# JCBrouwer/maua-style

Hardware: AMD Instinct MI355X
Metric: optimizer iterations/sec at 1024x1024 VGG-19 (higher is better)
Workload: dtype f32 (fp16x3 split-precision MFMA, fp32 accumulate)

## Files before the change

maua-style_amd/csrc/conv_x3p.hip:

```cpp
#include <stdlib.h>

#include <type_traits>

#include "conv_host.hpp"
#include "fp16x3.hpp"

namespace maua {

constexpr int XP_COT = 64;
constexpr int XP_ROWS = 16, XP_PR = 18, XP_PC = 34;
constexpr int XP_NPOS = XP_PR * XP_PC;
constexpr int XP_NPOS_PAD = 624;
constexpr int XP_PLANE = XP_NPOS_PAD * 16;
constexpr int XP_PATCH_BYTES = 8 * XP_PLANE;
constexpr int XP_TAP_BYTES = 2 * 4 * XP_COT * 16;
constexpr int XP_W_BYTES = 9 * XP_TAP_BYTES;
constexpr int XP_NI = 5;
constexpr int XP_THREADS = 512;
constexpr int XP_BIAS_MAX = 512;
constexpr int XP_LDS_BYTES = XP_PATCH_BYTES + XP_W_BYTES + 64 + XP_BIAS_MAX * 4 + XP_THREADS * 12;
constexpr unsigned XP_OOB = 0x80000000u;
#ifndef XP_W1_PIECES
#define XP_W1_PIECES 4
#endif
#ifndef XP_EARLY_LOADS
#define XP_EARLY_LOADS 0
#endif
#ifndef XP_MIDFOLD
#define XP_MIDFOLD 1
#endif
#ifndef XP_STAGGER
#define XP_STAGGER 0
#endif

__host__ __device__ constexpr int xp_first_pieces(bool pool) { return pool ? XP_W1_PIECES / 2 : XP_W1_PIECES; }
__host__ __device__ constexpr int xp_step_of(bool pool, int k) {
    const int p1 = xp_first_pieces(pool);
    return pool ? (k < p1 ? 16 - 2 * (p1 - 1 - k) : 20 + 2 * (k - p1)) : (k < p1 ? 17 - p1 + k : 20 + (k - p1));
}

struct X3pArgs {
    int items;
    int tiles;
    int ncot;
    int ksplit;
    int cps;
    int nmain;
    int n2;
    int groups;
    int tiles_y;
    int d_split, d_tx, d_ty, d_cot, d_n;
    int order;
    float w_inv_scale;
};

#ifdef XP_STAMP
#define XP_MARK(k)                                                                                                       \
    do {                                                                                                                 \
        if (lane == 0 && p.mask && chunk_no < 60) {                                                                      \
            const_cast<float*>(p.mask)[(((int64_t)blockIdx.x * 8 + wave) * 64 + chunk_no) * 8 + (k)] =                   \
                __builtin_bit_cast(float, (unsigned)__builtin_amdgcn_s_memtime());                                       \
        }                                                                                                                \
    } while (0)
#else
#define XP_MARK(k) do {} while (0)
#endif

#define XP_FENCE() __builtin_amdgcn_sched_barrier(0)

#define XP_PIPE_PLAIN(VA)                                             \
    do {                                                              \
        _Pragma("unroll") for (int m_ = 0; m_ < 12; ++m_) {           \
            __builtin_amdgcn_sched_group_barrier(0x008, 1, 0);        \
            __builtin_amdgcn_sched_group_barrier(0x100, 1, 0);        \
            __builtin_amdgcn_sched_group_barrier(0x020, 1, 0);        \
            __builtin_amdgcn_sched_group_barrier(0x200, 1, 0);        \
            __builtin_amdgcn_sched_group_barrier(0x002, VA, 0);       \
        }                                                             \
    } while (0)
#define XP_PIPE(VA)                                                   \
    do {                                                              \
        _Pragma("unroll") for (int m_ = 0; m_ < 12; ++m_) {           \
            __builtin_amdgcn_sched_group_barrier(0x008, 1, 0);        \
            __builtin_amdgcn_sched_group_barrier(0x100, 1, 0);        \
            __builtin_amdgcn_sched_group_barrier(0x020, 1, 0);        \
            __builtin_amdgcn_sched_group_barrier(0x040, 1, 0);        \
            __builtin_amdgcn_sched_group_barrier(0x200, 1, 0);        \
            __builtin_amdgcn_sched_group_barrier(0x002, VA, 0);       \
        }                                                             \
    } while (0)

template <bool OM, bool POOL, bool UNPOOL, bool GRAM>
__global__ void __launch_bounds__(XP_THREADS, 2) conv_x3p_kernel(ConvArgs p, X3pArgs q) {
    extern __shared__ __attribute__((aligned(16))) unsigned char smem[];
    unsigned char* Pl = smem;
    unsigned char* Wl = smem + XP_PATCH_BYTES;
    float* Ml = reinterpret_cast<float*>(smem + XP_PATCH_BYTES + XP_W_BYTES);
    float* Bl = Ml + 16;
    unsigned* Tl = reinterpret_cast<unsigned*>(Bl + XP_BIAS_MAX);

    const int tid = threadIdx.x;
    const int lane = tid & 63, wave = tid >> 6;
    const int px = lane & 15, oct = lane >> 4;
    const int wv = __builtin_amdgcn_readfirstlane(wave);
    auto my_tid = [&]() {
        int t = tid;
        asm volatile("" : "+v"(t));
        return t;
    };
    const float w_inv_scale = q.w_inv_scale;
    const int ksplit = q.ksplit;
    const bool slab = ksplit > 1;
    const int in_plane = p.H * p.W;
    const int out_plane = p.OH * p.OW;
    const int st_w = UNPOOL ? p.W >> 1 : p.W;
    const int st_plane = UNPOOL ? (p.H >> 1) * (p.W >> 1) : in_plane;
    const unsigned code_mask = (unsigned)p.in_code_mask;

    const int stride = q.groups >> 3;
    const int band_begin = (int)((int64_t)(blockIdx.x & 7) * q.items / 8), band_end = (int)((int64_t)((blockIdx.x & 7) + 1) * q.items / 8);
    const int gq = (int)(blockIdx.x & 7) * stride + (int)(blockIdx.x >> 3);
    const int item_begin = band_begin + (int)(blockIdx.x >> 3), item_end = band_end;
    if (item_begin >= item_end) return;
    if (XP_STAGGER > 0)
        for (int i = 0; i < (gq & 3) * XP_STAGGER; ++i) __builtin_amdgcn_s_sleep(16);
    struct Item {
        int n, cot, split, x0, y0, cb, ce;
    };
    const int tiles_w = p.tiles_x * 32, tiles_h = (q.tiles / p.tiles_x) * XP_ROWS;
    auto chunk_range = [&](Item& it) {
        it.cb = it.split * q.cps;
        it.ce = min(q.nmain, it.cb + q.cps);
    };
    auto decode = [&](int idx) {
        Item it;
        int t = idx;
        it.split = t % ksplit;
        t /= ksplit;
        int tile;
        if (q.order) {
            it.cot = t % q.ncot;
            t /= q.ncot;
            tile = t % q.tiles;
            it.n = t / q.tiles;
        } else {
            tile = t % q.tiles;
            t /= q.tiles;
            it.cot = t % q.ncot;
            it.n = t / q.ncot;
        }
        it.x0 = (tile % p.tiles_x) * 32;
        it.y0 = (tile / p.tiles_x) * XP_ROWS;
        it.n = __builtin_amdgcn_readfirstlane(it.n);
        it.cot = __builtin_amdgcn_readfirstlane(it.cot);
        it.split = __builtin_amdgcn_readfirstlane(it.split);
        it.x0 = __builtin_amdgcn_readfirstlane(it.x0);
        it.y0 = __builtin_amdgcn_readfirstlane(it.y0);
        chunk_range(it);
        return it;
    };
    auto advance = [&](Item it) {
        int c;
        it.split += q.d_split;
        c = it.split >= ksplit ? 1 : 0;
        it.split -= c ? ksplit : 0;
        if (q.order) {
            it.cot += q.d_cot + c;
            c = it.cot >= q.ncot ? 1 : 0;
            it.cot -= c ? q.ncot : 0;
        }
        it.x0 += (q.d_tx + c) * 32;
        c = it.x0 >= tiles_w ? 1 : 0;
        it.x0 -= c ? tiles_w : 0;
        it.y0 += (q.d_ty + c) * XP_ROWS;
        c = it.y0 >= tiles_h ? 1 : 0;
        it.y0 -= c ? tiles_h : 0;
        if (!q.order) {
            it.cot += q.d_cot + c;
            c = it.cot >= q.ncot ? 1 : 0;
            it.cot -= c ? q.ncot : 0;
        }
        it.n += q.d_n + c;
        chunk_range(it);
        return it;
    };

    constexpr int NI = UNPOOL ? 2 : XP_NI;
    constexpr int NV = 2;
    unsigned voff[NV];
    unsigned lds_w[2] = {0u, 0u};
    unsigned vcode[UNPOOL ? 2 : 1], inmask[UNPOOL ? 2 : 1];
    if constexpr (UNPOOL) {
        constexpr int PR = XP_ROWS / 2 + 2, PCW = 18;
#pragma unroll
        for (int k = 0; k < 2; ++k) {
            const int idx = tid + XP_THREADS * k;
            const int o = idx / (PR * PCW);
            const int rem = idx - o * PR * PCW;
            const int pr = rem / PCW, pc = rem - pr * PCW;
            Tl[k * XP_THREADS + tid] = (unsigned)(pr | pc << 8 | o << 16 | (idx < 4 * PR * PCW ? 1 << 24 : 0));
        }
    } else {
        const int ra = tid / XP_PC, ca = tid - ra * XP_PC;
        Tl[tid] = (unsigned)(ra | ca << 8 | 1 << 24);
        const int o4 = tid / 100, pb = 512 + tid - o4 * 100;
        const int rb = pb / XP_PC, cb4 = pb - rb * XP_PC;
        Tl[XP_THREADS + tid] = (unsigned)(rb | cb4 << 8 | o4 << 16 | (tid < 400 ? 1 << 24 : 0));
        vcode[0] = inmask[0] = 0;
    }
    auto set_tile = [&](int x0, int y0) {
        const int tid = my_tid();
        if constexpr (UNPOOL) {
#pragma unroll
            for (int k = 0; k < NI; ++k) {
                const unsigned wh = Tl[k * XP_THREADS + tid];
                const int pr = (int)(wh & 0xffu), pc = (int)((wh >> 8) & 0xffu), o = (int)((wh >> 16) & 0xffu);
                const bool item = (wh >> 24) != 0;
                const int ppy = ((y0 - p.pad) >> 1) + pr, ppx = ((x0 - p.pad) >> 1) + pc;
                const bool ok = item & ((unsigned)ppy < (unsigned)(p.H >> 1)) & ((unsigned)ppx < (unsigned)st_w);
                const int pidx = ppy * st_w + ppx;
                voff[k] = ok ? (unsigned)(o * 8 * st_plane + pidx) * 4u : XP_OOB;
                vcode[k] = ok ? (unsigned)(o * st_plane + pidx) * 8u : XP_OOB;
                const int r0 = 2 * ppy - (y0 - p.pad), c0 = 2 * ppx - (x0 - p.pad);
                inmask[k] = 0;
#pragma unroll
                for (int qd = 0; qd < 4; ++qd) {
                    const int r = r0 + (qd >> 1), c = c0 + (qd & 1);
                    inmask[k] |= (item & ((unsigned)r < (unsigned)XP_PR) & ((unsigned)c < (unsigned)XP_PC)) ? 1u << qd : 0u;
                }
                lds_w[k] = (unsigned)(o * XP_PLANE + (r0 * XP_PC + c0) * 16);
            }
        } else {
#pragma unroll
            for (int k = 0; k < 2; ++k) {
                const unsigned wh = Tl[k * XP_THREADS + tid];
                const int r = (int)(wh & 0xffu), c = (int)((wh >> 8) & 0xffu), o = (int)((wh >> 16) & 0xffu);
                const int iy = y0 + r - p.pad, ix = x0 + c - p.pad;
                const bool ok = ((wh >> 24) != 0) & ((unsigned)iy < (unsigned)p.H) & ((unsigned)ix < (unsigned)p.W);
                const unsigned v = ok ? (unsigned)(o * 8 * in_plane + iy * p.W + ix) * 4u : XP_OOB;
                if (k == 0) voff[0] = v;
                else Tl[2 * XP_THREADS + tid] = v;
            }
        }
    };
    const unsigned range = (unsigned)st_plane * 128u;
    float rp[NI][8];
    u32x2 cd[NI];
    unsigned sel2[NI][4];
    struct PatchSrc {
        __amdgpu_buffer_rsrc_t x, codes;
    };
    auto patch_rsrc = [&](int n, int ch) {
        asm volatile("" : "+s"(ch));
        PatchSrc r;
        const int64_t first = ((int64_t)n * p.Cin + (int64_t)ch * 32) * st_plane;
        r.x = __builtin_amdgcn_make_buffer_rsrc(const_cast<float*>(p.x + first), 0, range, 0x00020000);
        r.codes = r.x;
        if constexpr (UNPOOL) r.codes = __builtin_amdgcn_make_buffer_rsrc(const_cast<unsigned char*>(p.in_codes + first), 0, range >> 2, 0x00020000);
        return r;
    };
    auto load_patch_part = [&](const PatchSrc& rs, int c_lo, int c_hi) {
        if constexpr (UNPOOL) {
            if (c_lo == 0) {
#pragma unroll
                for (int k = 0; k < NI; ++k) cd[k] = __builtin_amdgcn_raw_buffer_load_b64(rs.codes, vcode[k], 0, 0);
            }
#pragma unroll
            for (int c = c_lo; c < c_hi; ++c)
#pragma unroll
                for (int k = 0; k < NI; ++k)
                    rp[k][c] = __builtin_bit_cast(float, __builtin_amdgcn_raw_buffer_load_b32(rs.x, voff[k], c * st_plane * 4, 0));
        } else {
#pragma unroll
            for (int c = c_lo; c < c_hi; ++c)
#pragma unroll
                for (int k = 0; k < NI; ++k)
                    rp[k][c] = __builtin_bit_cast(float, __builtin_amdgcn_raw_buffer_load_b32(rs.x, k < 4 ? voff[0] : voff[1], ((k < 4 ? 8 * k : 0) + c) * st_plane * 4, 0));
        }
    };
    auto publish_max = [&]() {
        if constexpr (UNPOOL) {
            const unsigned m2 = code_mask * 0x00010001u;
#pragma unroll
            for (int k = 0; k < NI; ++k)
#pragma unroll
                for (int i = 0; i < 4; ++i) {
                    sel2[k][i] = __builtin_amdgcn_perm(0u, cd[k][i >> 1], (i & 1) ? 0x0c030c02u : 0x0c010c00u) & m2;
                    const unsigned s0 = sel2[k][i] & 0xffffu, s1 = sel2[k][i] >> 16;
                    rp[k][2 * i] = ((inmask[k] >> s0) & 1u) ? rp[k][2 * i] : 0.f;
                    rp[k][2 * i + 1] = ((inmask[k] >> s1) & 1u) ? rp[k][2 * i + 1] : 0.f;
                }
        }
        float m = 0.f;
#pragma unroll
        for (int k = 0; k < NI; ++k)
#pragma unroll
            for (int c = 0; c < 8; ++c) m = fmaxf(m, fabsf(rp[k][c]));
        m = wave_max_nonneg(m);
        if ((my_tid() & 63) == 0) Ml[wv] = m;
    };
    float sx = 1.f;
    auto chunk_scale = [&]() {
        const float m = fmaxf(fmaxf(fmaxf(Ml[0], Ml[1]), fmaxf(Ml[2], Ml[3])), fmaxf(fmaxf(Ml[4], Ml[5]), fmaxf(Ml[6], Ml[7])));
        int e = (int)((__builtin_bit_cast(unsigned, m) >> 23) & 0xffu) - 127;
        e = m > 0.f ? max(e, -100) : 11;
        e = __builtin_amdgcn_readfirstlane(e);
        sx = __builtin_bit_cast(float, (unsigned)(127 + 11 - e) << 23);
        return __builtin_bit_cast(float, (unsigned)(127 + e - 11) << 23);
    };
    auto split_item = [&](int k) {
        if (k >= NI) return;
#pragma unroll
        for (int c = 0; c < 8; ++c) asm volatile("" : "+v"(rp[k][c]));
        unsigned hu[4], lu[4];
#pragma unroll
        for (int qd = 0; qd < 4; ++qd) {
            const float v0 = rp[k][2 * qd], v1 = rp[k][2 * qd + 1];
            const f16x2 h2 = {(_Float16)(v0 * sx), (_Float16)(v1 * sx)};
            const f16x2 l2 = {(_Float16)fmaf(v0, sx, -(float)h2[0]), (_Float16)fmaf(v1, sx, -(float)h2[1])};
            hu[qd] = __builtin_bit_cast(unsigned, h2);
            lu[qd] = __builtin_bit_cast(unsigned, l2);
        }
#pragma unroll
        for (int qd = 0; qd < 4; ++qd) {
            rp[k][qd] = __builtin_bit_cast(float, hu[qd]);
            rp[k][4 + qd] = __builtin_bit_cast(float, lu[qd]);
        }
#pragma unroll
        for (int c = 0; c < 8; ++c) asm volatile("" : "+v"(rp[k][c]));
    };
    auto store_patch = [&]() {
        if constexpr (UNPOOL) {
#pragma unroll
            for (int k = 0; k < NI; ++k)
#pragma unroll
                for (int qd = 0; qd < 4; ++qd)
                    if ((inmask[k] >> qd) & 1u) {
                        const unsigned dst = lds_w[k] + (unsigned)(((qd >> 1) * XP_PC + (qd & 1)) * 16);
                        u32x4 h, l;
#pragma unroll
                        for (int i = 0; i < 4; ++i) {
                            const unsigned t = sel2[k][i] ^ ((unsigned)qd * 0x00010001u);
                            const unsigned keep = ((t & 0xffffu) ? 0u : 0xffffu) | ((t >> 16) ? 0u : 0xffff0000u);
                            h[i] = __builtin_bit_cast(unsigned, rp[k][i]) & keep;
                            l[i] = __builtin_bit_cast(unsigned, rp[k][4 + i]) & keep;
                        }
                        *reinterpret_cast<u32x4*>(Pl + dst) = h;
                        *reinterpret_cast<u32x4*>(Pl + 4 * XP_PLANE + dst) = l;
                    }
            return;
        }
        const int t_ = my_tid();
#pragma unroll
        for (int k = 0; k < NI; ++k) {
            const u32x4 h = {__builtin_bit_cast(unsigned, rp[k][0]), __builtin_bit_cast(unsigned, rp[k][1]), __builtin_bit_cast(unsigned, rp[k][2]),
                             __builtin_bit_cast(unsigned, rp[k][3])};
            const u32x4 l = {__builtin_bit_cast(unsigned, rp[k][4]), __builtin_bit_cast(unsigned, rp[k][5]), __builtin_bit_cast(unsigned, rp[k][6]),
                             __builtin_bit_cast(unsigned, rp[k][7])};
            unsigned dst = (unsigned)t_ * 16u + (unsigned)(XP_PLANE * k);
            if (k == NI - 1) {
                const unsigned wh = Tl[XP_THREADS + t_];
                dst = (wh >> 24) ? ((wh >> 16) & 0xffu) * XP_PLANE + ((wh & 0xffu) * XP_PC + ((wh >> 8) & 0xffu)) * 16u : (unsigned)(3 * XP_PLANE + (XP_NPOS_PAD - 1) * 16);
            }
            *reinterpret_cast<u32x4*>(Pl + dst) = h;
            *reinterpret_cast<u32x4*>(Pl + 4 * XP_PLANE + dst) = l;
        }
    };

    const unsigned char* __restrict__ bank = reinterpret_cast<const unsigned char*>(p.w6);
    const unsigned lane16 = lane * 16;
    auto dma_filters = [&](int ch, int cot, int first, int count, int i0 = 0) {
        const unsigned char* src = bank + ((int64_t)ch * q.ncot + cot) * XP_W_BYTES;
#pragma unroll
        for (int i = i0; i < i0 + count; ++i) {
            const int pl = first + wv + 8 * i;
            const unsigned char* g = src + pl * 1024;
            const unsigned lds_dst = (unsigned)(size_t)(__attribute__((address_space(3))) unsigned char*)(Wl + pl * 1024);
            unsigned keep;
            asm volatile("s_mov_b32 %0, m0\n\ts_mov_b32 m0, %2\n\ts_nop 0\n\tglobal_load_lds_dwordx4 %1, %3\n\ts_mov_b32 m0, %0"
                         : "=&s"(keep)
                         : "v"(lane16), "s"(__builtin_amdgcn_readfirstlane(lds_dst)), "s"(g)
                         : "memory");
        }
    };

    int b_base = oct * XP_PLANE + ((2 * wave) * XP_PC + px) * 16;
    int a_base = oct * 1024 + px * 16;

    f32x4 acc[4][4], master[4][4];
    f16x8 bf[4][2], af[2][2];
    auto load_bg = [&](int g, int part, int tap) {
        const int ky = tap / 3, kx = tap - 3 * ky;
        bf[g][part] = *reinterpret_cast<const f16x8*>(Pl + b_base + part * 4 * XP_PLANE + (((g >> 1) + ky) * XP_PC + (g & 1) * 16 + kx) * 16);
    };
    auto load_ai = [&](int buf, int tap, int i) {
#pragma unroll
        for (int part = 0; part < 2; ++part) af[buf][part] = *reinterpret_cast<const f16x8*>(Wl + a_base + (tap * 2 + part) * 4096 + i * 256);
    };
    auto step_ = [&](auto stores, int tap, int i, int next_tap, auto fresh, float inv, auto va, auto&& extra) {
        constexpr bool FRESH = decltype(fresh)::value;
        constexpr int VA = decltype(va)::value;
        const int cur = i & 1;
        const bool refresh = i == 3 && next_tap >= 0;
        XP_FENCE();
        if (i < 3) load_ai(cur ^ 1, tap, i + 1);
        else if (next_tap >= 0 && tap != 4) load_ai(cur ^ 1, next_tap, 0);
        const f32x4 zero = {0.f, 0.f, 0.f, 0.f};
        if constexpr (FRESH) {
#pragma unroll
            for (int g = 0; g < 4; ++g) asm volatile("" : "+v"(acc[i][g]));
#pragma unroll
            for (int g = 0; g < 4; ++g)
#pragma unroll
                for (int r = 0; r < 4; ++r) master[i][g][r] = fmaf(acc[i][g][r], inv, master[i][g][r]);
#pragma unroll
            for (int g = 0; g < 4; ++g) asm volatile("" : "+v"(master[i][g]));
        }
#pragma unroll
        for (int g = 0; g < 4; ++g) acc[i][g] = __builtin_amdgcn_mfma_f32_16x16x32_f16(af[cur][1], bf[g][0], FRESH ? zero : acc[i][g], 0, 0, 0);
#pragma unroll
        for (int g = 0; g < 4; ++g) {
            acc[i][g] = __builtin_amdgcn_mfma_f32_16x16x32_f16(af[cur][0], bf[g][0], acc[i][g], 0, 0, 0);
            if (refresh) load_bg(g, 0, next_tap);
        }
        extra();
#pragma unroll
        for (int g = 0; g < 4; ++g) {
            acc[i][g] = __builtin_amdgcn_mfma_f32_16x16x32_f16(af[cur][0], bf[g][1], acc[i][g], 0, 0, 0);
            if (refresh) load_bg(g, 1, next_tap);
        }
        if constexpr (decltype(stores)::value) XP_PIPE(VA);
        else XP_PIPE_PLAIN(VA);
        XP_FENCE();
    };
    auto nothing = []() {};
    constexpr std::true_type FOLD{};
    constexpr std::false_type KEEP{};
    constexpr std::integral_constant<int, 0> V0{};
    constexpr std::integral_constant<int, 2> V2{};
    constexpr std::integral_constant<int, 4> V4{};

    Item cur = decode(item_begin);
    Item fin = cur;
    bool fin_valid = false;
    __amdgpu_buffer_rsrc_t rs_out, rs_aux;
    unsigned so_base = 0;
    unsigned vo[2];
    bool row_ok[4] = {true, true, true, true};
    const int PW = p.OW >> 1;
    const int pplane = (p.OH >> 1) * PW;
    auto epi_begin = [&]() {
        const int t_ = my_tid();
        const int lane = t_ & 63, px = t_ & 15, oct = (t_ >> 4) & 3, wave = wv;
        if constexpr (POOL) {
            const int64_t img = (int64_t)fin.n * p.Cout * pplane;
            rs_out = __builtin_amdgcn_make_buffer_rsrc(p.y + img, 0, (unsigned)p.Cout * (unsigned)pplane * 4u, 0x00020000);
            rs_aux = __builtin_amdgcn_make_buffer_rsrc(p.pool_codes + img, 0, (unsigned)p.Cout * (unsigned)pplane, 0x00020000);
            so_base = (unsigned)((fin.y0 >> 1) * PW + (fin.x0 >> 1));
#pragma unroll
            for (int h = 0; h < 2; ++h) {
                const int oy = fin.y0 + 2 * wave, oxx = fin.x0 + 16 * h + px;
                const bool store = fin_valid && (lane & 1) == 0 && oy + 1 < p.OH && oxx + 1 < p.OW;
                vo[h] = store ? (unsigned)(wave * PW + ((16 * h + px) >> 1)) : XP_OOB;
            }
        } else {
            const int64_t img = (int64_t)fin.n * p.Cout * out_plane;
            float* base = slab ? p.ws + ((int64_t)fin.n * ksplit + fin.split) * p.Cout * out_plane : p.y + img;
            rs_out = __builtin_amdgcn_make_buffer_rsrc(base, 0, (unsigned)p.Cout * (unsigned)out_plane * 4u, 0x00020000);
            rs_aux = rs_out;
            if constexpr (OM) rs_aux = __builtin_amdgcn_make_buffer_rsrc(const_cast<float*>(p.omask + img), 0, (unsigned)p.Cout * (unsigned)out_plane * 4u, 0x00020000);
            so_base = (unsigned)((fin.cot * XP_COT) * out_plane + fin.y0 * p.OW + fin.x0) * 4u;
#pragma unroll
            for (int h = 0; h < 2; ++h)
                vo[h] = fin_valid && fin.x0 + 16 * h + px < p.OW ? (unsigned)((4 * oct) * out_plane + (2 * wave) * p.OW + 16 * h + px) * 4u : XP_OOB;
#pragma unroll
            for (int g = 0; g < 4; ++g) row_ok[g] = fin.y0 + 2 * wv + (g >> 1) < p.OH;
        }
    };
    float mk[2][4];
    auto epi_load = [&](int k) {
        if constexpr (OM) {
            const int i = k >> 2, g = k & 3;
            const unsigned v = row_ok[g] ? vo[g & 1] : XP_OOB;
#pragma unroll
            for (int r = 0; r < 4; ++r)
                mk[k % 2][r] = __builtin_bit_cast(float, __builtin_amdgcn_raw_buffer_load_b32(
                    rs_aux, v, so_base + (unsigned)((16 * i + r) * out_plane + (g >> 1) * p.OW) * 4u, 0));
        }
    };
    auto reset_group = [&](int i, int cot) {
        const int oct = (my_tid() >> 4) & 3;
        const f32x4 b = *reinterpret_cast<const f32x4*>(Bl + cot * XP_COT + 16 * i + 4 * oct);
#pragma unroll
        for (int g = 0; g < 4; ++g) master[i][g] = b;
    };
    auto epi_piece = [&](int k, int next_cot) {
        const int oct = (my_tid() >> 4) & 3;
        if constexpr (POOL) {
            if (k >= 8) return;
            const int i = k >> 1, h = k & 1;
            unsigned pk = 0;
            const unsigned so = (unsigned)((fin.cot * XP_COT + 16 * i) * pplane) + so_base;
#pragma unroll
            for (int r = 0; r < 4; ++r) {
                float a = master[i][h][r], c = master[i][2 + h][r];
                a = a > 0.f ? a : 0.f;
                c = c > 0.f ? c : 0.f;
                const float b = __builtin_bit_cast(float, __builtin_amdgcn_update_dpp(0, __builtin_bit_cast(int, a), 0x101, 0xf, 0xf, false));
                const float d = __builtin_bit_cast(float, __builtin_amdgcn_update_dpp(0, __builtin_bit_cast(int, c), 0x101, 0xf, 0xf, false));
                float m = a;
                unsigned arg = 0;
                if (b > m) { m = b; arg = 1; }
                if (c > m) { m = c; arg = 2; }
                if (d > m) { m = d; arg = 3; }
                pk |= (arg | (m > 0.f ? 0u : 4u)) << (8 * r);
                const unsigned v = vo[h] == XP_OOB ? XP_OOB : ((unsigned)(4 * oct * pplane) + vo[h]) * 4u;
                __builtin_amdgcn_raw_buffer_store_b32(__builtin_bit_cast(unsigned, m), rs_out, v, (so + (unsigned)(r * pplane)) * 4u, 0);
            }
            const unsigned vc = vo[h] == XP_OOB ? XP_OOB : ((unsigned)((oct >> 1) * pplane) + vo[h]) * 8u + 4u * (oct & 1);
            __builtin_amdgcn_raw_buffer_store_b32(pk, rs_aux, vc, ((unsigned)(((fin.cot * XP_COT + 16 * i) >> 3) * pplane) + so_base) * 8u, 0);
            if (h == 1) reset_group(i, next_cot);
        } else {
            const int i = k >> 2, g = k & 3;
            const unsigned v = row_ok[g] ? vo[g & 1] : XP_OOB;
#pragma unroll
            for (int r = 0; r < 4; ++r) {
                float val = master[i][g][r];
                if (p.relu && !slab) val = val > 0.f ? val : 0.f;
                if constexpr (OM) val = mk[k % 2][r] > 0.f ? val : 0.f;
                __builtin_amdgcn_raw_buffer_store_b32(__builtin_bit_cast(unsigned, val), rs_out, v,
                                                      so_base + (unsigned)((16 * i + r) * out_plane + (g >> 1) * p.OW) * 4u, 0);
            }
            if (g == 3) reset_group(i, next_cot);
        }
    };

    auto gram_phase = [&](const Item& it, float inv_pending) {
#pragma unroll
        for (int i = 0; i < 4; ++i)
#pragma unroll
            for (int g = 0; g < 4; ++g)
#pragma unroll
                for (int r = 0; r < 4; ++r) {
                    master[i][g][r] = fmaf(acc[i][g][r], inv_pending, master[i][g][r]);
                    acc[i][g][r] = 0.f;
                }
        const float d_inv_scale = p.dinv[it.n];
        const unsigned char* dbank = reinterpret_cast<const unsigned char*>(p.dbank);
        unsigned vf[4];
#pragma unroll
        for (int g = 0; g < 4; ++g) {
            const int oy = it.y0 + 2 * wave + (g >> 1), oxx = it.x0 + (g & 1) * 16 + px;
            vf[g] = (oy < p.OH && oxx < p.OW) ? (unsigned)((oct * 8) * out_plane + oy * p.OW + oxx) * 4u : XP_OOB;
        }
        const unsigned frange = (unsigned)out_plane * 128u;
        float f[4][8];
        auto request = [&](int c2) {
            asm volatile("" : "+s"(c2));
            const __amdgpu_buffer_rsrc_t rs = __builtin_amdgcn_make_buffer_rsrc(
                const_cast<float*>(p.omask + ((int64_t)it.n * p.Cout + (int64_t)c2 * 32) * out_plane), 0, frange, 0x00020000);
#pragma unroll
            for (int c = 0; c < 8; ++c)
#pragma unroll
                for (int g = 0; g < 4; ++g) f[g][c] = __builtin_bit_cast(float, __builtin_amdgcn_raw_buffer_load_b32(rs, vf[g], c * out_plane * 4, 0));
        };
        request(0);
        for (int c2 = 0; c2 < q.n2; ++c2) {
            float m = 0.f;
#pragma unroll
            for (int g = 0; g < 4; ++g)
#pragma unroll
                for (int c = 0; c < 8; ++c) m = fmaxf(m, fabsf(f[g][c]));
            m = wave_max_nonneg(m);
            int e = (int)((__builtin_bit_cast(unsigned, m) >> 23) & 0xffu) - 127;
            e = m > 0.f ? max(e, -100) : 11;
            const float s = __builtin_bit_cast(float, (unsigned)(127 + 11 - e) << 23);
            const float inv = __builtin_bit_cast(float, (unsigned)(127 + e - 11) << 23) * d_inv_scale;
            f16x8 b[4][2];
#pragma unroll
            for (int g = 0; g < 4; ++g) {
                u32x4 Hh, Ll;
#pragma unroll
                for (int qd = 0; qd < 4; ++qd) {
                    const float v0 = f[g][2 * qd], v1 = f[g][2 * qd + 1];
                    const f16x2 h2 = {(_Float16)(v0 * s), (_Float16)(v1 * s)};
                    const f16x2 l2 = {(_Float16)fmaf(v0, s, -(float)h2[0]), (_Float16)fmaf(v1, s, -(float)h2[1])};
                    Hh[qd] = __builtin_bit_cast(unsigned, h2);
                    Ll[qd] = __builtin_bit_cast(unsigned, l2);
                }
                b[g][0] = __builtin_bit_cast(f16x8, Hh);
                b[g][1] = __builtin_bit_cast(f16x8, Ll);
            }
            const unsigned char* gsrc = dbank + ((((int64_t)it.n * (2 * q.n2) + 2 * c2 + (oct >> 1)) * q.ncot + it.cot) * 4096) + (oct & 1) * 1024 + px * 16;
            u32x4 a[4][2];
#pragma unroll
            for (int i = 0; i < 4; ++i)
#pragma unroll
                for (int part = 0; part < 2; ++part) a[i][part] = *reinterpret_cast<const u32x4*>(gsrc + part * 2048 + i * 256);
            if (c2 + 1 < q.n2) request(c2 + 1);
#pragma unroll
            for (int i = 0; i < 4; ++i) {
                const f16x8 ah = __builtin_bit_cast(f16x8, a[i][0]), al = __builtin_bit_cast(f16x8, a[i][1]);
#pragma unroll
                for (int g = 0; g < 4; ++g) {
                    acc[i][g] = __builtin_amdgcn_mfma_f32_16x16x32_f16(al, b[g][0], acc[i][g], 0, 0, 0);
                    acc[i][g] = __builtin_amdgcn_mfma_f32_16x16x32_f16(ah, b[g][1], acc[i][g], 0, 0, 0);
                    acc[i][g] = __builtin_amdgcn_mfma_f32_16x16x32_f16(ah, b[g][0], acc[i][g], 0, 0, 0);
                }
            }
#pragma unroll
            for (int i = 0; i < 4; ++i)
#pragma unroll
                for (int g = 0; g < 4; ++g)
#pragma unroll
                    for (int r = 0; r < 4; ++r) {
                        master[i][g][r] = fmaf(acc[i][g][r], inv, master[i][g][r]);
                        acc[i][g][r] = 0.f;
                    }
        }
    };

    for (int c = tid; c < p.Cout; c += XP_THREADS) Bl[c] = (p.bias != nullptr && !slab) ? p.bias[c] : 0.f;
    set_tile(cur.x0, cur.y0);
    int ch = cur.cb;
    dma_filters(ch, cur.cot, 0, 9);
    if constexpr (!UNPOOL) voff[1] = Tl[2 * XP_THREADS + tid];
    load_patch_part(patch_rsrc(cur.n, ch), 0, 8);
    publish_max();
    asm volatile("s_waitcnt lgkmcnt(0)" ::: "memory");
    __builtin_amdgcn_s_barrier();
    float inv_prev = 0.f, inv_cur = 0.f, inv_next = 0.f;
    inv_cur = chunk_scale() * w_inv_scale;
    inv_next = inv_cur;
#pragma unroll
    for (int k = 0; k < NI; ++k) split_item(k);
    store_patch();
#pragma unroll
    for (int i = 0; i < 4; ++i) {
        reset_group(i, cur.cot);
#pragma unroll
        for (int g = 0; g < 4; ++g) acc[i][g] = f32x4{0.f, 0.f, 0.f, 0.f};
    }
    asm volatile("s_waitcnt vmcnt(0) lgkmcnt(0)" ::: "memory");
    __builtin_amdgcn_s_barrier();

#ifdef XP_STAMP
    int chunk_no = 0;
#endif
    auto chunk_body = [&](auto epi_tag, const Item& it, int chn, bool later, bool more, const Item& nx, int nch, const PatchSrc& rs) {
        constexpr bool EPI = decltype(epi_tag)::value;
        auto step = [&](int tap, int i, int next_tap, auto fresh, float inv, auto va, auto&& extra) {
            step_(std::integral_constant<bool, EPI>{}, tap, i, next_tap, fresh, inv, va, extra);
        };
        {
            const int t_ = my_tid();
            if constexpr (!UNPOOL) voff[1] = Tl[2 * XP_THREADS + t_];
            b_base = ((t_ >> 4) & 3) * XP_PLANE + ((2 * wv) * XP_PC + (t_ & 15)) * 16;
            a_base = ((t_ >> 4) & 3) * 1024 + (t_ & 15) * 16;
        }
        const int ncot_ = it.cot;
        if constexpr (EPI) epi_begin();
        constexpr int NP = POOL ? 8 : 16;
        constexpr int P1 = xp_first_pieces(POOL);
        auto step_of = [](int k) { return xp_step_of(POOL, k); };
        auto E = [&](int s) {
            if constexpr (EPI) {
#pragma unroll
                for (int k = 0; k < NP; ++k) {
                    if constexpr (OM) {
                        if (k < 1 ? s == step_of(0) - 1 : s == step_of(k - 1)) epi_load(k);
                    }
                }
#pragma unroll
                for (int k = 0; k < NP; ++k)
                    if (s == step_of(k) && fin_valid) epi_piece(k, ncot_);
            }
        };
        constexpr int SPP = POOL ? 5 : 4;
        constexpr int ST1 = !EPI ? 0 : SPP * P1;
        constexpr int late2 = POOL ? (NP - P1 > 3 ? NP - P1 - 3 : 0) : (NP - P1 > 5 ? NP - P1 - 5 : 0);
        constexpr int ST2 = !EPI ? 0 : SPP * late2;
        static_assert(ST1 <= 60 && ST2 <= 60 && xp_step_of(POOL, NP - 1) <= 31 && xp_step_of(POOL, 0) >= 5, "conv_x3p: epilogue schedule");
        constexpr std::integral_constant<int, EPI ? 4 : 2> VF{};
        constexpr std::integral_constant<int, EPI ? 2 : 0> VK{};
        XP_MARK(0);
#pragma unroll
        for (int g = 0; g < 4; ++g) {
            load_bg(g, 0, 0);
            load_bg(g, 1, 0);
        }
        load_ai(0, 0, 0);
        if constexpr (EPI || XP_EARLY_LOADS) {
            step(0, 0, 1, FOLD, inv_prev, VF, [&]() { load_patch_part(rs, 0, 1); });
            step(0, 1, 1, FOLD, inv_prev, VF, [&]() { load_patch_part(rs, 1, 2); if (later) dma_filters(chn, it.cot, 40, 1, 0); });
            step(0, 2, 1, FOLD, inv_prev, VF, [&]() { load_patch_part(rs, 2, 3); });
            step(0, 3, 1, FOLD, inv_prev, VF, [&]() { load_patch_part(rs, 3, 4); if (later) dma_filters(chn, it.cot, 40, 1, 1); });
            step(1, 0, 2, KEEP, 0.f, VK, [&]() { load_patch_part(rs, 4, 5); E(4); });
            step(1, 1, 2, KEEP, 0.f, VK, [&]() { load_patch_part(rs, 5, 6); if (later) dma_filters(chn, it.cot, 40, 1, 2); E(5); });
            step(1, 2, 2, KEEP, 0.f, VK, [&]() { load_patch_part(rs, 6, 7); E(6); });
            step(1, 3, 2, KEEP, 0.f, VK, [&]() { load_patch_part(rs, 7, 8); if (later) dma_filters(chn, it.cot, 40, 1, 3); E(7); });
#pragma unroll
            for (int tap = 2; tap < 4; ++tap)
#pragma unroll
                for (int i = 0; i < 4; ++i) step(tap, i, tap + 1, KEEP, 0.f, VK, [&]() { E(4 * tap + i); });
        } else {
            step(0, 0, 1, FOLD, inv_prev, VF, [&]() { load_patch_part(rs, 0, 1); });
            step(0, 1, 1, FOLD, inv_prev, VF, nothing);
            step(0, 2, 1, FOLD, inv_prev, VF, [&]() { load_patch_part(rs, 1, 2); });
            step(0, 3, 1, FOLD, inv_prev, VF, [&]() { if (later) dma_filters(chn, it.cot, 40, 1, 0); });
#pragma unroll
            for (int tap = 1; tap < 4; ++tap) {
                step(tap, 0, tap + 1, KEEP, 0.f, VK, [&]() { load_patch_part(rs, 2 * tap, 2 * tap + 1); });
                step(tap, 1, tap + 1, KEEP, 0.f, VK, nothing);
                step(tap, 2, tap + 1, KEEP, 0.f, VK, [&]() { load_patch_part(rs, 2 * tap + 1, 2 * tap + 2); });
                step(tap, 3, tap + 1, KEEP, 0.f, VK, [&]() { if (later) dma_filters(chn, it.cot, 40, 1, tap); });
            }
        }
        XP_MARK(1);
        step(4, 0, 5, KEEP, 0.f, VK, [&]() { E(16); });
        if (EPI && fin_valid) asm volatile("s_waitcnt vmcnt(%0)" ::"n"(ST1) : "memory");
        else asm volatile("s_waitcnt vmcnt(0)" ::: "memory");
        step(4, 1, 5, KEEP, 0.f, V4, [&]() { publish_max(); });
        step(4, 2, 5, KEEP, 0.f, V4, nothing);
        step(4, 3, 5, KEEP, 0.f, V0, nothing);
        XP_MARK(2);
        if (EPI && fin_valid) asm volatile("s_waitcnt vmcnt(%0) lgkmcnt(0)" ::"n"(ST1) : "memory");
        else asm volatile("s_waitcnt vmcnt(0) lgkmcnt(0)" ::: "memory");
        __builtin_amdgcn_s_barrier();
        XP_MARK(3);
        load_ai(0, 5, 0);
        inv_next = chunk_scale() * w_inv_scale;
        if constexpr (EPI) {
            step(5, 0, 6, KEEP, 0.f, V2, [&]() { if (more) dma_filters(nch, nx.cot, 0, 1, 0); E(20); });
            step(5, 1, 6, KEEP, 0.f, V2, [&]() { if (more) dma_filters(nch, nx.cot, 0, 1, 1); E(21); });
            step(5, 2, 6, KEEP, 0.f, V2, [&]() { if (more) dma_filters(nch, nx.cot, 0, 1, 2); E(22); });
            step(5, 3, 6, KEEP, 0.f, V2, [&]() { if (more) dma_filters(nch, nx.cot, 0, 1, 3); E(23); });
            step(6, 0, 7, KEEP, 0.f, V4, [&]() { if (more) dma_filters(nch, nx.cot, 0, 1, 4); split_item(0); E(24); });
            step(6, 1, 7, KEEP, 0.f, V4, [&]() { split_item(1); E(25); });
            step(6, 2, 7, KEEP, 0.f, V4, [&]() { split_item(2); E(26); });
            step(6, 3, 7, KEEP, 0.f, V4, [&]() { split_item(3); E(27); });
            step(7, 0, 8, KEEP, 0.f, V4, [&]() { split_item(4); E(28); });
            step(7, 1, 8, KEEP, 0.f, V2, [&]() { E(29); });
            step(7, 2, 8, KEEP, 0.f, V2, [&]() { E(30); });
            step(7, 3, 8, KEEP, 0.f, V2, [&]() { E(31); });
            step(8, 0, -1, KEEP, 0.f, V0, nothing);
            step(8, 1, -1, KEEP, 0.f, V0, nothing);
            step(8, 2, -1, KEEP, 0.f, V0, nothing);
            step(8, 3, -1, KEEP, 0.f, V0, nothing);
        } else {
            constexpr std::integral_constant<bool, XP_MIDFOLD != 0> MID{};
            step(5, 0, 6, MID, inv_cur, V2, nothing);
            step(5, 1, 6, MID, inv_cur, V2, [&]() { if (more) dma_filters(nch, nx.cot, 0, 1, 0); });
            step(5, 2, 6, MID, inv_cur, V2, nothing);
            step(5, 3, 6, MID, inv_cur, V2, [&]() { if (more) dma_filters(nch, nx.cot, 0, 1, 1); });
            step(6, 0, 7, KEEP, 0.f, V4, [&]() { split_item(0); });
            step(6, 1, 7, KEEP, 0.f, V4, [&]() { split_item(1); });
            step(6, 2, 7, KEEP, 0.f, V4, [&]() { split_item(2); });
            step(6, 3, 7, KEEP, 0.f, V0, [&]() { if (more) dma_filters(nch, nx.cot, 0, 1, 2); });
            step(7, 0, 8, KEEP, 0.f, V4, [&]() { split_item(3); });
            step(7, 1, 8, KEEP, 0.f, V4, [&]() { split_item(4); });
            step(7, 2, 8, KEEP, 0.f, V0, nothing);
            step(7, 3, 8, KEEP, 0.f, V0, [&]() { if (more) dma_filters(nch, nx.cot, 0, 1, 3); });
            step(8, 0, -1, KEEP, 0.f, V0, nothing);
            step(8, 1, -1, KEEP, 0.f, V0, [&]() { if (more) dma_filters(nch, nx.cot, 0, 1, 4); });
            step(8, 2, -1, KEEP, 0.f, V0, nothing);
            step(8, 3, -1, KEEP, 0.f, V0, nothing);
        }
        XP_MARK(4);
        inv_prev = inv_cur;
        inv_cur = inv_next;
        asm volatile("s_waitcnt lgkmcnt(0)" ::: "memory");
        __builtin_amdgcn_s_barrier();
        XP_MARK(5);
        store_patch();
        if (EPI && fin_valid) asm volatile("s_waitcnt vmcnt(%0) lgkmcnt(0)" ::"n"(ST2) : "memory");
        else asm volatile("s_waitcnt vmcnt(0) lgkmcnt(0)" ::: "memory");
        __builtin_amdgcn_s_barrier();
        XP_MARK(6);
#ifdef XP_STAMP
        XP_MARK(7);
        ++chunk_no;
#endif
    };

    int item = item_begin;
    bool later = false;
    Item nx = cur;
    int nch = 0;
    bool more = true;
    PatchSrc rs;
    auto plan_next = [&](int chn) {
        const bool last_of_item = chn + 1 >= cur.ce;
        more = !(last_of_item && item + stride >= item_end);
        nx = cur;
        nch = chn + 1;
        if (last_of_item && more) {
            nx = advance(cur);
            nch = nx.cb;
            set_tile(nx.x0, nx.y0);
        }
        rs = patch_rsrc(more ? nx.n : cur.n, more ? nch : chn);
    };
    while (true) {
        plan_next(cur.cb);
        chunk_body(std::true_type{}, cur, cur.cb, later, more, nx, nch, rs);
        later = true;
        for (int chn = cur.cb + 1; chn < cur.ce; ++chn) {
            plan_next(chn);
            chunk_body(std::false_type{}, cur, chn, later, more, nx, nch, rs);
        }
        if constexpr (GRAM) {
            if (cur.split == ksplit - 1) {
                gram_phase(cur, inv_prev);
                inv_prev = 0.f;
            }
        }
        fin = cur;
        fin_valid = true;
        item += stride;
        if (!more) break;
        cur = nx;
    }
#pragma unroll
    for (int i = 0; i < 4; ++i)
#pragma unroll
        for (int g = 0; g < 4; ++g)
#pragma unroll
            for (int r = 0; r < 4; ++r) master[i][g][r] = fmaf(acc[i][g][r], inv_prev, master[i][g][r]);
    epi_begin();
    if constexpr (POOL) {
#pragma unroll
        for (int k = 0; k < 8; ++k) epi_piece(k, fin.cot);
    } else {
#pragma unroll
        for (int i = 0; i < 4; ++i) {
#pragma unroll
            for (int g = 0; g < 4; ++g) {
                epi_load(4 * i + g);
                epi_piece(4 * i + g, fin.cot);
            }
        }
    }
}


static int x3p_choose_split(const ConvArgs& a) {
    const int64_t items = conv_tiles(a, XP_ROWS) * ((a.Cout + XP_COT - 1) / XP_COT) * split_batch_hint();
    const int nchunks = a.Cin / 32;
    const int forced = (int)tuning("x3p_ks", 0);
    auto whole = [&](int ks) { const int cps = (nchunks + ks - 1) / ks; return (nchunks + cps - 1) / cps; };
    if (nchunks < 1) return 1;
    if (forced > 0) return whole(forced <= nchunks / 2 ? forced : (nchunks >= 4 ? nchunks / 2 : 1));
    if (items >= 512 || nchunks < 4) return 1;
    const double out_mb = (double)split_batch_hint() * a.Cout * a.OH * a.OW * 4.0 / 1e6;
    int best = 1;
    double best_cost = 1e30;
    for (int ks = 1; ks <= 16 && ks <= nchunks / 2; ++ks) {
        const int64_t its = items * ks;
        const double per_wg = (double)((its + 255) / 256);
        double cost = (per_wg * (double)((nchunks + ks - 1) / ks) + 0.7) * 9.0;
        if (ks > 1) cost += (ks + 1) * out_mb / 5.0 + 5.0;
        if (cost < best_cost * 0.97) {
            best_cost = cost;
            best = ks;
        }
    }
    return whole(best);
}

bool conv_x3p_supports(const ConvArgs& a) {
    return a.Cin % 32 == 0 && a.Cout % XP_COT == 0 && a.Cout <= XP_BIAS_MAX && (int64_t)a.H * a.W <= (1ll << 24) && a.pad >= 0 && a.pad <= 2 &&
           (int64_t)a.Cout * a.OH * a.OW * 4 < (1ll << 31) && (int64_t)a.OH * a.OW <= (1ll << 24);
}

static int g_xp_max_groups = 0;
static int x3p_max_groups() {
    const int v = g_xp_max_groups > 0 ? g_xp_max_groups : (int)tuning("x3p_groups", 256);
    return v >= 8 ? v / 8 * 8 : 256;
}

#ifdef XP_STAMP
static float* g_xp_stamp = nullptr;
extern "C" void maua_xp_set_stamp_buffer(float* buf) { g_xp_stamp = buf; }
#endif

template <bool OM, bool POOL, bool UNPOOL, bool GRAM>
static int xp_launch_one(const ConvArgs& p, const X3pArgs& q, hipStream_t stream) {
    const void* fn = reinterpret_cast<const void*>(&conv_x3p_kernel<OM, POOL, UNPOOL, GRAM>);
    static unsigned long long served = 0;
    const hipError_t rc = opt_in_dynamic_lds(fn, XP_LDS_BYTES, &served);
    if (rc != hipSuccess) {
        set_error("conv_x3p: hipFuncSetAttribute: %s", hipGetErrorString(rc));
        return (int)rc;
    }
    hipLaunchKernelGGL((conv_x3p_kernel<OM, POOL, UNPOOL, GRAM>), dim3((unsigned)q.groups), dim3(XP_THREADS), XP_LDS_BYTES, stream, p, q);
    return check_launch("conv_x3p_kernel");
}

int conv_x3p_launch(const ConvArgs& a, int n, float w_scale, hipStream_t stream) {
    ConvArgs p = a;
#ifdef XP_STAMP
    p.mask = g_xp_stamp;
#endif
    p.tiles_x = (a.OW + 31) / 32;
    X3pArgs q{};
    q.tiles = p.tiles_x * ((a.OH + XP_ROWS - 1) / XP_ROWS);
    q.ncot = a.Cout / XP_COT;
    const int ks = a.ws ? x3p_choose_split(a) : 1;
    q.ksplit = ks;
    p.ksplit = ks;
    q.nmain = a.Cin / 32;
    q.cps = (q.nmain + ks - 1) / ks;
    q.n2 = a.dbank ? a.Cout / 32 : 0;
    const int64_t items = (int64_t)n * q.ncot * q.tiles * ks;
    if (items > (1ll << 30)) {
        set_error("conv_x3p: too many work items");
        return MAUA_E_UNSUPPORTED;
    }
    q.items = (int)items;
    const int max_groups = x3p_max_groups();
    q.groups = (int)(items >= max_groups ? max_groups : (items + 7) / 8 * 8);
    q.tiles_y = q.tiles / p.tiles_x;
    q.order = tuning("x3p_order", 1) != 0 ? 1 : 0;
    {
        int st = q.groups / 8;
        q.d_split = st % ks;
        st /= ks;
        if (q.order) {
            q.d_cot = st % q.ncot;
            st /= q.ncot;
        }
        q.d_tx = st % p.tiles_x;
        st /= p.tiles_x;
        q.d_ty = st % q.tiles_y;
        st /= q.tiles_y;
        if (q.order) {
            q.d_n = st;
        } else {
            q.d_cot = st % q.ncot;
            q.d_n = st / q.ncot;
        }
    }
    q.w_inv_scale = 1.f / w_scale;
    const bool om = ks == 1 && a.omask != nullptr, gram = a.dbank != nullptr, unpool = a.in_codes != nullptr;
    int rc;
    if (a.pool_codes && ks == 1) rc = xp_launch_one<false, true, false, false>(p, q, stream);
    else if (unpool && gram && om) rc = xp_launch_one<true, false, true, true>(p, q, stream);
    else if (unpool && gram) rc = xp_launch_one<false, false, true, true>(p, q, stream);
    else if (unpool && om) rc = xp_launch_one<true, false, true, false>(p, q, stream);
    else if (unpool) rc = xp_launch_one<false, false, true, false>(p, q, stream);
    else if (gram && om) rc = xp_launch_one<true, false, false, true>(p, q, stream);
    else if (gram) rc = xp_launch_one<false, false, false, true>(p, q, stream);
    else if (om) rc = xp_launch_one<true, false, false, false>(p, q, stream);
    else rc = xp_launch_one<false, false, false, false>(p, q, stream);
    if (rc || ks == 1) return rc;
    return a.pool_codes ? conv_splitk_finish_pool(a, n, ks, stream) : conv_splitk_finish(a, n, ks, stream);
}

}

using namespace maua;

extern "C" {

int maua_conv_x3p_supported(int cin, int h, int w, int cout, int pad) {
    ConvArgs a;
    return conv_geometry(a, 1, cin, h, w, cout, 3, pad) == CONV_SHAPE_OK && conv_x3p_supports(a) ? 1 : 0;
}

int maua_conv_x3p_split(int n, int cin, int h, int w, int cout, int pad) {
    ConvArgs a;
    return conv_geometry(a, n, cin, h, w, cout, 3, pad) == CONV_SHAPE_OK ? x3p_choose_split(a) : 0;
}

static size_t x3p_workspace_bytes(const ConvArgs& a, int n) {
    const int ks = x3p_choose_split(a);
    return ks > 1 ? (size_t)n * ks * a.Cout * a.OH * a.OW * sizeof(float) : 0;
}
size_t maua_conv_x3p_workspace_bytes(int n, int cin, int h, int w, int cout, int pad) {
    ConvArgs a;
    return conv_geometry(a, n, cin, h, w, cout, 3, pad) == CONV_SHAPE_OK ? x3p_workspace_bytes(a, n) : 0;
}

int maua_conv_x3p_set_max_groups(int groups) {
    const int before = g_xp_max_groups;
    g_xp_max_groups = groups >= 8 ? groups / 8 * 8 : 0;
    return before;
}

int maua_conv_x3p_preferred(int n, int cin, int h, int w, int cout, int pad) {
    ConvArgs a;
    if (conv_geometry(a, n, cin, h, w, cout, 3, pad) != CONV_SHAPE_OK || !conv_x3p_supports(a)) return 0;
    const int oh = a.OH, ow = a.OW;
    const double min_fill = tuning("x3p_min_fill", 0.8);
    const int min_items = (int)tuning("x3p_min_items", 512);
    const int ks = x3p_choose_split(a);
    const int64_t items = conv_tiles(a, XP_ROWS) * (cout / XP_COT) * split_batch_hint() * ks;
    const double fill = (double)items / (double)(((items + 255) / 256) * 256);
    const double cover = (double)oh * ow / ((double)((oh + XP_ROWS - 1) / XP_ROWS * XP_ROWS) * ((ow + 31) / 32 * 32));
    return ks == 1 && items >= min_items && items * (cin / 32) >= 4 * (int64_t)min_items && fill * cover >= min_fill ? 1 : 0;
}

int maua_conv3x3_x3p(const float* x, const unsigned char* in_codes, int honour_relu_bit, const void* bank, float w_scale, const float* bias,
                     const float* out_relu_mask, const void* dmat_bank, const float* dmat_inv_scale, float* y, unsigned char* pool_codes,
                     int n, int cin, int h, int w, int cout, int pad, int relu, void* workspace, size_t workspace_bytes, maua_stream_t stream) {
    MAUA_REQUIRE(x && bank && y && w_scale > 0.f, MAUA_E_INVAL, "conv3x3_x3p: bad args");
    ConvArgs a;
    const ConvShape shape = conv_geometry(a, n, cin, h, w, cout, 3, pad);
    MAUA_REQUIRE(shape != CONV_SHAPE_BAD_DIMS && pad <= 2, MAUA_E_INVAL, "conv3x3_x3p: bad dims");
    MAUA_REQUIRE(shape == CONV_SHAPE_OK, MAUA_E_UNSUPPORTED, "conv3x3_x3p: input smaller than the filter");
    a.x = x;
    a.w6 = bank;
    a.bias = bias;
    a.omask = out_relu_mask;
    a.y = y;
    a.relu = relu;
    MAUA_REQUIRE(conv_x3p_supports(a), MAUA_E_UNSUPPORTED,
                 "conv3x3_x3p: needs cin %% 32 == 0, cout %% 64 == 0, cout <= 512, planes of at most 2^24 pixels and an output image below 2 GiB");
    if (pool_codes) {
        MAUA_REQUIRE(a.OH >= 2 && a.OW >= 2 && !out_relu_mask && !dmat_bank && !in_codes && relu, MAUA_E_UNSUPPORTED,
                     "conv3x3_x3p: the pooling form is conv + bias + ReLU + pool of an output plane of 2 x 2 and more");
        a.pool_codes = pool_codes;
    }
    if (dmat_bank) {
        MAUA_REQUIRE(dmat_inv_scale && out_relu_mask, MAUA_E_INVAL, "conv3x3_x3p: the Gram term needs the feature map and the bank's inverse scale");
        MAUA_REQUIRE(a.OH == h && a.OW == w, MAUA_E_UNSUPPORTED, "conv3x3_x3p: the Gram term needs an output plane of the input's size");
        a.dbank = dmat_bank;
        a.dinv = dmat_inv_scale;
    }
    if (in_codes) {
        MAUA_REQUIRE(h >= 2 && w >= 2, MAUA_E_UNSUPPORTED, "conv3x3_x3p: the unpooling form needs an input plane of 2 x 2 and more");
        a.in_codes = in_codes;
        a.in_code_mask = honour_relu_bit ? 7 : 3;
    }
    size_t need = 0;
    accept_workspace(a, workspace, workspace_bytes, false, [&] { return need = x3p_workspace_bytes(a, n); });
    if (need == 0) a.ws = nullptr;
    return conv_x3p_launch(a, n, w_scale, (hipStream_t)stream);
}

}
```

Baseline: 202.9.

## Prefetch output-mask into packed bits during last K-chunk of conv kernel

Adds a BITS kernel variant used for masked (ReLU-backward style) convolutions without Gram. It peels the last input-channel chunk so the output-mask loads are issued during that chunk's MFMA steps. The loaded values are packed into two 32-bit bitmasks, so the epilogue only tests bits instead of waiting on mask loads. It also recomputes unpool code offsets and LDS write addresses on demand from the LDS table to lower register pressure. The cost is a more complex schedule, extra instructions in the last chunk, and a larger temporary mask array.

```diff
diff --git a/maua-style_amd/csrc/conv_x3p.hip b/maua-style_amd/csrc/conv_x3p.hip
--- a/maua-style_amd/csrc/conv_x3p.hip
+++ b/maua-style_amd/csrc/conv_x3p.hip
@@ -32,8 +32,15 @@
 #ifndef XP_STAGGER
 #define XP_STAGGER 0
 #endif
+#ifndef XP_MASK_BITS
+#define XP_MASK_BITS 1
+#endif
 
 __host__ __device__ constexpr int xp_first_pieces(bool pool) { return pool ? XP_W1_PIECES / 2 : XP_W1_PIECES; }
+__host__ __device__ constexpr int xp_mask_step(bool unpool, int k) { return unpool ? 3 * (k / 4) + (k / 2) % 2 : k < 4 ? 0 : k < 8 ? 1 : k < 12 ? 4 : k < 14 ? 5 : 8; }
+__host__ __device__ constexpr int xp_mask_lat(bool unpool) { return unpool ? 3 : 4; }
+__host__ __device__ constexpr int xp_mask_slot(bool unpool, int k) { return unpool ? k % 4 : k < 8 ? k : k < 14 ? k - 8 : k - 14; }
+__host__ __device__ constexpr int xp_last_patch_step(bool unpool, int c) { return unpool ? (c < 7 ? 8 + c : 14) : c < 4 ? 4 + 2 * c : 7 + c; }
 __host__ __device__ constexpr int xp_step_of(bool pool, int k) {
     const int p1 = xp_first_pieces(pool);
     return pool ? (k < p1 ? 16 - 2 * (p1 - 1 - k) : 20 + 2 * (k - p1)) : (k < p1 ? 17 - p1 + k : 20 + (k - p1));
@@ -90,7 +97,7 @@
         }                                                             \
     } while (0)
 
-template <bool OM, bool POOL, bool UNPOOL, bool GRAM>
+template <bool OM, bool POOL, bool UNPOOL, bool GRAM, bool BITS = false>
 __global__ void __launch_bounds__(XP_THREADS, 2) conv_x3p_kernel(ConvArgs p, X3pArgs q) {
     extern __shared__ __attribute__((aligned(16))) unsigned char smem[];
     unsigned char* Pl = smem;
@@ -220,7 +227,7 @@
                 const bool ok = item & ((unsigned)ppy < (unsigned)(p.H >> 1)) & ((unsigned)ppx < (unsigned)st_w);
                 const int pidx = ppy * st_w + ppx;
                 voff[k] = ok ? (unsigned)(o * 8 * st_plane + pidx) * 4u : XP_OOB;
-                vcode[k] = ok ? (unsigned)(o * st_plane + pidx) * 8u : XP_OOB;
+                if constexpr (!BITS) vcode[k] = ok ? (unsigned)(o * st_plane + pidx) * 8u : XP_OOB;
                 const int r0 = 2 * ppy - (y0 - p.pad), c0 = 2 * ppx - (x0 - p.pad);
                 inmask[k] = 0;
 #pragma unroll
@@ -228,7 +235,7 @@
                     const int r = r0 + (qd >> 1), c = c0 + (qd & 1);
                     inmask[k] |= (item & ((unsigned)r < (unsigned)XP_PR) & ((unsigned)c < (unsigned)XP_PC)) ? 1u << qd : 0u;
                 }
-                lds_w[k] = (unsigned)(o * XP_PLANE + (r0 * XP_PC + c0) * 16);
+                if constexpr (!BITS) lds_w[k] = (unsigned)(o * XP_PLANE + (r0 * XP_PC + c0) * 16);
             }
         } else {
 #pragma unroll
@@ -262,6 +269,14 @@
     auto load_patch_part = [&](const PatchSrc& rs, int c_lo, int c_hi) {
         if constexpr (UNPOOL) {
             if (c_lo == 0) {
+                if constexpr (BITS) {
+                    const int t_ = my_tid();
+#pragma unroll
+                    for (int k = 0; k < NI; ++k) {
+                        const unsigned o = (Tl[k * XP_THREADS + t_] >> 16) & 0xffu;
+                        vcode[k] = voff[k] == XP_OOB ? XP_OOB : 2u * voff[k] - 56u * o * (unsigned)st_plane;
+                    }
+                }
 #pragma unroll
                 for (int k = 0; k < NI; ++k) cd[k] = __builtin_amdgcn_raw_buffer_load_b64(rs.codes, vcode[k], 0, 0);
             }
@@ -331,6 +346,16 @@
     };
     auto store_patch = [&]() {
         if constexpr (UNPOOL) {
+            if constexpr (BITS) {
+                const int t_ = my_tid();
+#pragma unroll
+                for (int k = 0; k < NI; ++k) {
+                    const unsigned wh = Tl[k * XP_THREADS + t_];
+                    const int pr = (int)(wh & 0xffu), pc = (int)((wh >> 8) & 0xffu), o = (int)((wh >> 16) & 0xffu);
+                    const int r0 = 2 * pr - (p.pad & 1), c0 = 2 * pc - (p.pad & 1);
+                    lds_w[k] = (unsigned)(o * XP_PLANE + (r0 * XP_PC + c0) * 16);
+                }
+            }
 #pragma unroll
             for (int k = 0; k < NI; ++k)
 #pragma unroll
@@ -477,14 +502,21 @@
             for (int g = 0; g < 4; ++g) row_ok[g] = fin.y0 + 2 * wv + (g >> 1) < p.OH;
         }
     };
-    float mk[2][4];
+    float mk[BITS ? 8 : 2][4];
+    auto mslot = [](int k) { return BITS ? xp_mask_slot(UNPOOL, k) : k % 2; };
+    unsigned mbits[2] = {0u, 0u};
+    auto mask_bits = [&](int k) {
+#pragma unroll
+        for (int r = 0; r < 4; ++r) mbits[k >> 3] |= mk[mslot(k)][r] > 0.f ? 1u << (4 * (k & 7) + r) : 0u;
+        asm volatile("" : "+v"(mbits[k >> 3]));
+    };
     auto epi_load = [&](int k) {
         if constexpr (OM) {
             const int i = k >> 2, g = k & 3;
             const unsigned v = row_ok[g] ? vo[g & 1] : XP_OOB;
 #pragma unroll
             for (int r = 0; r < 4; ++r)
-                mk[k % 2][r] = __builtin_bit_cast(float, __builtin_amdgcn_raw_buffer_load_b32(
+                mk[mslot(k)][r] = __builtin_bit_cast(float, __builtin_amdgcn_raw_buffer_load_b32(
                     rs_aux, v, so_base + (unsigned)((16 * i + r) * out_plane + (g >> 1) * p.OW) * 4u, 0));
         }
     };
@@ -527,7 +559,8 @@
             for (int r = 0; r < 4; ++r) {
                 float val = master[i][g][r];
                 if (p.relu && !slab) val = val > 0.f ? val : 0.f;
-                if constexpr (OM) val = mk[k % 2][r] > 0.f ? val : 0.f;
+                if constexpr (BITS) val = ((mbits[k >> 3] >> (4 * (k & 7) + r)) & 1u) ? val : 0.f;
+                else if constexpr (OM) val = mk[mslot(k)][r] > 0.f ? val : 0.f;
                 __builtin_amdgcn_raw_buffer_store_b32(__builtin_bit_cast(unsigned, val), rs_out, v,
                                                       so_base + (unsigned)((16 * i + r) * out_plane + (g >> 1) * p.OW) * 4u, 0);
             }
@@ -647,8 +680,9 @@
 #ifdef XP_STAMP
     int chunk_no = 0;
 #endif
-    auto chunk_body = [&](auto epi_tag, const Item& it, int chn, bool later, bool more, const Item& nx, int nch, const PatchSrc& rs) {
-        constexpr bool EPI = decltype(epi_tag)::value;
+    auto chunk_body = [&](auto form_tag, const Item& it, int chn, bool later, bool more, const Item& nx, int nch, const PatchSrc& rs) {
+        constexpr bool EPI = decltype(form_tag)::value == 1;
+        constexpr bool LASTC = BITS && decltype(form_tag)::value == 2;
         auto step = [&](int tap, int i, int next_tap, auto fresh, float inv, auto va, auto&& extra) {
             step_(std::integral_constant<bool, EPI>{}, tap, i, next_tap, fresh, inv, va, extra);
         };
@@ -660,14 +694,26 @@
         }
         const int ncot_ = it.cot;
         if constexpr (EPI) epi_begin();
+        if constexpr (LASTC) {
+            epi_begin();
+            mbits[0] = mbits[1] = 0u;
+        }
         constexpr int NP = POOL ? 8 : 16;
         constexpr int P1 = xp_first_pieces(POOL);
         auto step_of = [](int k) { return xp_step_of(POOL, k); };
         auto E = [&](int s) {
+            if constexpr (LASTC) {
+#pragma unroll
+                for (int k = 0; k < 16; ++k)
+                    if (s == xp_mask_step(UNPOOL, k) + xp_mask_lat(UNPOOL)) mask_bits(k);
+#pragma unroll
+                for (int k = 0; k < 16; ++k)
+                    if (s == xp_mask_step(UNPOOL, k)) epi_load(k);
+            }
             if constexpr (EPI) {
 #pragma unroll
                 for (int k = 0; k < NP; ++k) {
-                    if constexpr (OM) {
+                    if constexpr (OM && !BITS) {
                         if (k < 1 ? s == step_of(0) - 1 : s == step_of(k - 1)) epi_load(k);
                     }
                 }
@@ -682,7 +728,7 @@
         constexpr int ST2 = !EPI ? 0 : SPP * late2;
         static_assert(ST1 <= 60 && ST2 <= 60 && xp_step_of(POOL, NP - 1) <= 31 && xp_step_of(POOL, 0) >= 5, "conv_x3p: epilogue schedule");
         constexpr std::integral_constant<int, EPI ? 4 : 2> VF{};
-        constexpr std::integral_constant<int, EPI ? 2 : 0> VK{};
+        constexpr std::integral_constant<int, EPI ? 2 : LASTC ? 4 : 0> VK{};
         XP_MARK(0);
 #pragma unroll
         for (int g = 0; g < 4; ++g) {
@@ -703,6 +749,20 @@
             for (int tap = 2; tap < 4; ++tap)
 #pragma unroll
                 for (int i = 0; i < 4; ++i) step(tap, i, tap + 1, KEEP, 0.f, VK, [&]() { E(4 * tap + i); });
+        } else if constexpr (LASTC) {
+            auto rides = [&](int st) {
+#pragma unroll
+                for (int c = 0; c < 8; ++c)
+                    if (xp_last_patch_step(UNPOOL, c) == st) load_patch_part(rs, c, c + 1);
+                if ((st & 3) == 3 && later) dma_filters(chn, it.cot, 40, 1, st >> 2);
+                E(st);
+            };
+#pragma unroll
+            for (int i = 0; i < 4; ++i) step(0, i, 1, FOLD, inv_prev, VF, [&]() { rides(i); });
+#pragma unroll
+            for (int tap = 1; tap < 4; ++tap)
+#pragma unroll
+                for (int i = 0; i < 4; ++i) step(tap, i, tap + 1, KEEP, 0.f, VK, [&]() { rides(4 * tap + i); });
         } else {
             step(0, 0, 1, FOLD, inv_prev, VF, [&]() { load_patch_part(rs, 0, 1); });
             step(0, 1, 1, FOLD, inv_prev, VF, nothing);
@@ -803,11 +863,17 @@
     };
     while (true) {
         plan_next(cur.cb);
-        chunk_body(std::true_type{}, cur, cur.cb, later, more, nx, nch, rs);
+        chunk_body(std::integral_constant<int, 1>{}, cur, cur.cb, later, more, nx, nch, rs);
         later = true;
-        for (int chn = cur.cb + 1; chn < cur.ce; ++chn) {
+        for (int chn = cur.cb + 1; chn < (BITS ? cur.ce - 1 : cur.ce); ++chn) {
             plan_next(chn);
-            chunk_body(std::false_type{}, cur, chn, later, more, nx, nch, rs);
+            chunk_body(std::integral_constant<int, 0>{}, cur, chn, later, more, nx, nch, rs);
+        }
+        if constexpr (BITS) {
+            fin = cur;
+            fin_valid = true;
+            plan_next(cur.ce - 1);
+            chunk_body(std::integral_constant<int, 2>{}, cur, cur.ce - 1, later, more, nx, nch, rs);
         }
         if constexpr (GRAM) {
             if (cur.split == ksplit - 1) {
@@ -831,6 +897,9 @@
     if constexpr (POOL) {
 #pragma unroll
         for (int k = 0; k < 8; ++k) epi_piece(k, fin.cot);
+    } else if constexpr (BITS) {
+#pragma unroll
+        for (int k = 0; k < 16; ++k) epi_piece(k, fin.cot);
     } else {
 #pragma unroll
         for (int i = 0; i < 4; ++i) {
@@ -884,16 +953,16 @@
 extern "C" void maua_xp_set_stamp_buffer(float* buf) { g_xp_stamp = buf; }
 #endif
 
-template <bool OM, bool POOL, bool UNPOOL, bool GRAM>
+template <bool OM, bool POOL, bool UNPOOL, bool GRAM, bool BITS = false>
 static int xp_launch_one(const ConvArgs& p, const X3pArgs& q, hipStream_t stream) {
-    const void* fn = reinterpret_cast<const void*>(&conv_x3p_kernel<OM, POOL, UNPOOL, GRAM>);
+    const void* fn = reinterpret_cast<const void*>(&conv_x3p_kernel<OM, POOL, UNPOOL, GRAM, BITS>);
     static unsigned long long served = 0;
     const hipError_t rc = opt_in_dynamic_lds(fn, XP_LDS_BYTES, &served);
     if (rc != hipSuccess) {
         set_error("conv_x3p: hipFuncSetAttribute: %s", hipGetErrorString(rc));
         return (int)rc;
     }
-    hipLaunchKernelGGL((conv_x3p_kernel<OM, POOL, UNPOOL, GRAM>), dim3((unsigned)q.groups), dim3(XP_THREADS), XP_LDS_BYTES, stream, p, q);
+    hipLaunchKernelGGL((conv_x3p_kernel<OM, POOL, UNPOOL, GRAM, BITS>), dim3((unsigned)q.groups), dim3(XP_THREADS), XP_LDS_BYTES, stream, p, q);
     return check_launch("conv_x3p_kernel");
 }
 
@@ -943,14 +1012,22 @@
     }
     q.w_inv_scale = 1.f / w_scale;
     const bool om = ks == 1 && a.omask != nullptr, gram = a.dbank != nullptr, unpool = a.in_codes != nullptr;
+    const bool bits = XP_MASK_BITS != 0 && om && !gram && q.nmain >= 2;
+    (void)bits;
     int rc;
     if (a.pool_codes && ks == 1) rc = xp_launch_one<false, true, false, false>(p, q, stream);
     else if (unpool && gram && om) rc = xp_launch_one<true, false, true, true>(p, q, stream);
     else if (unpool && gram) rc = xp_launch_one<false, false, true, true>(p, q, stream);
+#if XP_MASK_BITS
+    else if (unpool && bits) rc = xp_launch_one<true, false, true, false, true>(p, q, stream);
+#endif
     else if (unpool && om) rc = xp_launch_one<true, false, true, false>(p, q, stream);
     else if (unpool) rc = xp_launch_one<false, false, true, false>(p, q, stream);
     else if (gram && om) rc = xp_launch_one<true, false, false, true>(p, q, stream);
     else if (gram) rc = xp_launch_one<false, false, false, true>(p, q, stream);
+#if XP_MASK_BITS
+    else if (bits) rc = xp_launch_one<true, false, false, false, true>(p, q, stream);
+#endif
     else if (om) rc = xp_launch_one<true, false, false, false>(p, q, stream);
     else rc = xp_launch_one<false, false, false, false>(p, q, stream);
     if (rc || ks == 1) return rc;
```

Result: no change. 203.6, median of 6 (+0.4%).
